# jacobnzw/SSMToybox

Measured on AMD Instinct MI355X. Metric: filter steps/sec (batched MC) for GPQ-Kalman UNGM, higher is better.
Workload: dtype f64; 1 GPU; GPQ-Kalman (GaussianProcessTransform, RBF, UT points) on UNGM, D=1, N=3, 10000 MC trajectories per GPU x T=100 per pass (BASELINE configs[1]); mc_per_gpu=10000, mc_total=10000, parallelism=mc-shard x1, collective=SingleComm, devices=1 x  (gfx950:sramecc+:xnack-, 256 CUs) [0000:8e:00.0], distinct_devices=1, comm_world=1

## Files before the change

include/ssmq.h:

```cpp
#ifndef SSMQ_H
#define SSMQ_H

#ifndef __HIPCC_RTC__
#include <stddef.h>
#include <stdint.h>
#endif

#ifdef __cplusplus
extern "C" {
#endif

#define SSMQ_VERSION 102

#define SSMQ_OK 0
#define SSMQ_E_ARG (-1)
#define SSMQ_E_HIP (-2)
#define SSMQ_E_UNSUPPORTED (-3)
#define SSMQ_E_NOMEM (-4)

#define SSMQ_MAX_FPAR 16
#define SSMQ_MAX_FIDX 16
#define SSMQ_MAX_DIM 16
#define SSMQ_MAX_PTS 4096

// ... 256 lines not shown
                      const int32_t *d_status, const double *mse, double *sums);

int ssmq_traj_scores_rows(int D);
int ssmq_traj_scores_dev(int D, int64_t B, int64_t ld, int T, int k0, const double *d_x, const double *d_fm, const double *d_fP,
                         const int32_t *d_status, const double *mse, double *d_scores);

int ssmq_bootstrap_var_dev(const double *d_data, int64_t ld, int R, const int32_t *d_idx, int64_t n, int S, uint64_t seed,
                           double *var, double *d_means);
int ssmq_bootstrap_var(const double *data, int64_t n, int S, uint64_t seed, double *var);

int ssmq_mc_transform_dev(const ssmq_integrand *f, int D, int E, int64_t n, uint64_t seed, int64_t B, int64_t ld,
                          const double *d_mean, const double *d_cov, const double *d_time, int time_stride, double *d_mean_f,
                          double *d_cov_f, double *d_cov_fx, int32_t *d_status);
int ssmq_mc_unit_points(int D, uint64_t seed, int64_t first, int64_t count, double *z);

int ssmq_kl_divergence_dev(int E, int64_t B, int64_t ld, const double *d_m0, const double *d_P0, int bcast0, const double *d_m1,
                           const double *d_P1, int symmetrized, double *d_kl, int32_t *d_status);

int ssmq_student_filter_forward_dev(ssmq_transform *h_dyn, const ssmq_integrand *f_dyn, ssmq_transform *h_obs,
                                    const ssmq_integrand *f_obs, int64_t B, int64_t ld, int T, const double *d_y,
                                    const double *d_m0, const double *d_S0, const double *GqG, const double *r_smat,
                                    const double *scale, double dof, double *d_fm, double *d_fP, int32_t *d_status);

typedef struct ssmq_filter_job {
    ssmq_transform *h_dyn;
    const ssmq_integrand *f_dyn;
    ssmq_transform *h_obs;
    const ssmq_integrand *f_obs;
    int64_t B, ld;
    int32_t T, reserved;
    const double *d_y, *d_m0, *d_P0;
    const double *GQG, *R;
    double *d_fm, *d_fP;
    int32_t *d_status;
    const double *scale;
    double dof;
} ssmq_filter_job;
int ssmq_filter_forward_multi_dev(int n_jobs, const ssmq_filter_job *jobs);

#define SSMQ_PIPED_OUT_PINNED 1
#define SSMQ_PIPED_X0_PER_TRAJECTORY 2
int ssmq_filter_forward_piped(ssmq_transform *h_dyn, const ssmq_integrand *f_dyn, ssmq_transform *h_obs,
                              const ssmq_integrand *f_obs, int64_t B, int T, const double *y, const double *m0,
                              const double *P0, const double *GQG, const double *R, double *fm, double *fP,
                              int32_t *status, int flags, int n_blocks);
int ssmq_pinned_alloc(size_t bytes, void **p);
int ssmq_pinned_free(void *p);
int ssmq_pinned_is_block(const void *p);

int ssmq_filter_kernel_name(const ssmq_transform *h_dyn, const ssmq_integrand *f_dyn, const ssmq_transform *h_obs,
                            const ssmq_integrand *f_obs, char *buf, int len);
int ssmq_filter_kernel_name_batch(const ssmq_transform *h_dyn, const ssmq_integrand *f_dyn, const ssmq_transform *h_obs,
                                  const ssmq_integrand *f_obs, int64_t B, char *buf, int len);

int ssmq_filter_innovations_dev(ssmq_transform *h_dyn, const ssmq_integrand *f_dyn, ssmq_transform *h_obs,
                                const ssmq_integrand *f_obs, int64_t B, int64_t ld, int T, const double *d_y, const double *d_m0,
                                const double *d_P0, const double *d_fm, const double *d_fP, const double *GQG, const double *R,
                                double *d_ymean, double *d_S, double *d_nis, double *d_ll, double *d_total, int32_t *d_status);
int ssmq_innovations_kernel_name(const ssmq_transform *h_dyn, const ssmq_integrand *f_dyn, const ssmq_transform *h_obs,
                                 const ssmq_integrand *f_obs, int64_t B, char *buf, int len);

#define SSMQ_ITERATED_MAX 64
#define SSMQ_ITERATED_LAUNCH_LOOP 1
int ssmq_filter_iterated_dev(ssmq_transform *h_dyn, const ssmq_integrand *f_dyn, ssmq_transform *h_obs, const ssmq_integrand *f_obs,
                             int64_t B, int64_t ld, int T, int iterations, int flags, const double *d_y, const double *d_m0,
                             const double *d_P0, const double *GQG, const double *R, double *d_fm, double *d_fP,
                             double *d_delta , int32_t *d_status);
int ssmq_iterated_kernel_name(const ssmq_transform *h_dyn, const ssmq_integrand *f_dyn, const ssmq_transform *h_obs,
                              const ssmq_integrand *f_obs, int64_t B, int iterations, int flags, char *buf, int len);

int ssmq_smoother_iterated_dev(ssmq_transform *h_dyn, const ssmq_integrand *f_dyn, ssmq_transform *h_obs, const ssmq_integrand *f_obs,
                               int64_t B, int64_t ld, int T, const double *d_y, const double *d_m0, const double *d_P0,
                               const double *GQG, const double *R, int iterations, int flags,
                               const double *d_lin_m , const double *d_lin_P ,
                               double *d_fm, double *d_fP, double *d_sm, double *d_sP, double *d_sm0 ,
                               double *d_sP0 , double *d_delta , int32_t *d_status);
int ssmq_smoother_iterated_kernel_name(const ssmq_transform *h_dyn, const ssmq_integrand *f_dyn, const ssmq_transform *h_obs,
                                       const ssmq_integrand *f_obs, int iterations, char *buf, int len);

#define SSMQ_SWEEP_GP 0
#define SSMQ_SWEEP_BS 1
int ssmq_filter_sweep_dev(const ssmq_integrand *f_dyn, const ssmq_integrand *f_obs, int kind_dyn, int kind_obs, const double *xi_dyn,
                          int N_dyn, const double *xi_obs, int N_obs, const int32_t *mulind_dyn, int NB_dyn, const int32_t *mulind_obs,
                          int NB_obs, const double *par_dyn, const double *par_obs, int P, double jitter_dyn, double jitter_obs, int D,
                          int Y, int64_t B, int64_t ld, int T, const double *d_y, const double *x0_mean, const double *x0_cov,
                          const double *GQG, const double *R, double *d_loglik_total, double *d_nis_mean, double *d_loglik_steps,
                          int32_t *d_status, int32_t *theta_status);
int ssmq_filter_sweep_kernel_name(const ssmq_integrand *f_dyn, const ssmq_integrand *f_obs, int kind_dyn, int kind_obs, int N_dyn,
                                  int N_obs, int D, int Y, char *buf, int len);

int ssmq_student_scores_dev(ssmq_transform *h_dyn, const ssmq_integrand *f_dyn, ssmq_transform *h_obs, const ssmq_integrand *f_obs,
                            int64_t B, int64_t ld, int T, const double *d_y, const double *x0_mean, const double *x0_smat,
                            const double *GqG, const double *r_smat, const double *scale, double dof, double *d_nis, double *d_loglik,
                            double *d_loglik_total, double *d_nis_mean, int32_t *d_status);
int ssmq_student_scores_kernel_name(const ssmq_transform *h_dyn, const ssmq_integrand *f_dyn, const ssmq_transform *h_obs,
                                    const ssmq_integrand *f_obs, char *buf, int len);

#define SSMQ_RECURSION_GAUSS 0
#define SSMQ_RECURSION_STUDENT 1
int ssmq_filter_sweep_t_dev(const ssmq_integrand *f_dyn, const ssmq_integrand *f_obs, int recursion, const double *xi_dyn, int N_dyn,
                            const double *xi_obs, int N_obs, const double *par_dyn, const double *par_obs, const double *nu_dyn,
                            const double *nu_obs, const double *dof, int P, double jitter_dyn, double jitter_obs, int D, int Y, int64_t B,
                            int64_t ld, int T, const double *d_y, const double *x0_mean, const double *x0_mat, const double *GQG,
                            const double *R, const double *scale, double *d_loglik_total, double *d_nis_mean, double *d_loglik_steps,
                            int32_t *d_status, int32_t *theta_status);
int ssmq_filter_sweep_t_kernel_name(const ssmq_integrand *f_dyn, const ssmq_integrand *f_obs, int recursion, int N_dyn, int N_obs, int D,
// ... 63 lines not shown
```

ssmtoybox_amd/_lib.py:

```python
import ctypes
import os

import numpy as np

c_double_p = ctypes.POINTER(ctypes.c_double)
c_int32_p = ctypes.POINTER(ctypes.c_int32)

ABI_VERSION = 102
SSMQ_MAX_FPAR = 16
SSMQ_MAX_FIDX = 16
FORM_BQ, FORM_SIGMA = 0, 1
FORM_BQ_MO = 3
FORM_TAYLOR_GPQD = 4
FORM_TRUNC_SIGMA = 5
FORM_GPQD = 6
EMV_DIAG, EMV_BROADCAST = 0, 1

F_UNGM_DYN, F_UNGM_MEAS, F_UNGMNA_DYN, F_UNGMNA_MEAS = 1, 2, 3, 4
F_PENDULUM_DYN, F_PENDULUM_MEAS, F_REENTRY1D_DYN, F_RANGE_MEAS = 5, 6, 7, 8
F_REENTRY2D_DYN, F_RADAR2D_MEAS, F_CT_DYN, F_BEARING_MEAS = 9, 10, 11, 12
F_CTRS_DYN, F_CV_DYN, F_REENTRY2D_BIAS_DYN, F_SMOOTH10D_DYN = 13, 14, 15, 16
F_USER_FIRST, F_USER_SLOTS, USER_BODY_MAX, USER_MAX_D, USER_MAX_Y = 1024, 64, 8192, 6, 4
RTC_FILTER, RTC_APPLY, RTC_MC, RTC_LINEAR, RTC_TAYLOR_GPQD, RTC_GPQD, RTC_INNOVATION, RTC_ITERATED = 0, 1, 2, 3, 4, 5, 6, 7
RTC_SMOOTHER_ITERATED = 8
# ... 194 lines not shown
    'ssmq_particle_filter_dev': (ctypes.c_int, [ctypes.POINTER(Integrand), ctypes.POINTER(Integrand), ctypes.c_int, ctypes.c_int, ctypes.c_int,
                                                ctypes.c_int, ctypes.c_int64, ctypes.c_int64, ctypes.c_int] + [ctypes.c_void_p] * 3 +
                                 [c_double_p, c_double_p, c_double_p, ctypes.POINTER(Rv), ctypes.c_double, ctypes.c_uint64, ctypes.c_uint64] +
                                 [ctypes.c_void_p] * 8),
    'ssmq_particle_kernel_name': (ctypes.c_int, [ctypes.POINTER(Integrand), ctypes.POINTER(Integrand), ctypes.c_int, ctypes.c_int, ctypes.c_int,
                                                 ctypes.c_int, ctypes.POINTER(Rv), ctypes.c_char_p, ctypes.c_int]),
    'ssmq_particle_smoother_dev': (ctypes.c_int, [ctypes.POINTER(Integrand), ctypes.c_int, ctypes.c_int, ctypes.c_int, ctypes.c_int64,
                                                  ctypes.c_int64, ctypes.c_int, c_double_p, c_double_p, c_double_p, ctypes.c_int] +
                                   [ctypes.c_void_p] * 13),
    'ssmq_particle_smoother_kernel_name': (ctypes.c_int, [ctypes.POINTER(Integrand), ctypes.c_int, ctypes.c_int, ctypes.c_int, c_double_p,
                                                          c_double_p, c_double_p, ctypes.c_int, ctypes.c_char_p, ctypes.c_int]),
    'ssmq_particle_filter_rv_dev': (ctypes.c_int, [ctypes.POINTER(Integrand), ctypes.POINTER(Integrand), ctypes.c_int, ctypes.c_int, ctypes.c_int,
                                                   ctypes.c_int, ctypes.c_int64, ctypes.c_int64, ctypes.c_int] + [ctypes.c_void_p] * 3 +
                                    [ctypes.POINTER(Rv), ctypes.POINTER(Rv), c_double_p, ctypes.POINTER(Rv), ctypes.c_double, ctypes.c_uint64,
                                     ctypes.c_uint64] + [ctypes.c_void_p] * 8),
    'ssmq_particle_kernel_name_rv': (ctypes.c_int, [ctypes.POINTER(Integrand), ctypes.POINTER(Integrand), ctypes.c_int, ctypes.c_int, ctypes.c_int,
                                                    ctypes.c_int, ctypes.POINTER(Rv), ctypes.POINTER(Rv), ctypes.POINTER(Rv), ctypes.c_char_p,
                                                    ctypes.c_int]),
    'ssmq_particle_smoother_rv_dev': (ctypes.c_int, [ctypes.POINTER(Integrand), ctypes.c_int, ctypes.c_int, ctypes.c_int, ctypes.c_int64,
                                                     ctypes.c_int64, ctypes.c_int, ctypes.POINTER(Rv), c_double_p, ctypes.c_int] +
                                      [ctypes.c_void_p] * 13),
    'ssmq_particle_smoother_kernel_name_rv': (ctypes.c_int, [ctypes.POINTER(Integrand), ctypes.c_int, ctypes.c_int, ctypes.c_int,
                                                             ctypes.POINTER(Rv), c_double_p, ctypes.c_int, ctypes.c_char_p, ctypes.c_int]),
    'ssmq_pcrlb_sums_width': (ctypes.c_int, [ctypes.c_int]),
    'ssmq_pcrlb_sums_dev': (ctypes.c_int, [ctypes.POINTER(Integrand), ctypes.POINTER(Integrand), ctypes.c_int, ctypes.c_int, ctypes.c_int,
                                           ctypes.c_int64, ctypes.c_int64, ctypes.c_int, ctypes.c_void_p, ctypes.POINTER(Rv), c_double_p,
                                           ctypes.POINTER(Rv), c_double_p]),
    'ssmq_pcrlb_kernel_name': (ctypes.c_int, [ctypes.POINTER(Integrand), ctypes.POINTER(Integrand), ctypes.c_int, ctypes.c_int, ctypes.c_int,
                                              ctypes.POINTER(Rv), c_double_p, ctypes.POINTER(Rv), ctypes.c_char_p, ctypes.c_int]),
    'ssmq_pcrlb_finalize': (ctypes.c_int, [ctypes.c_int, ctypes.c_int, ctypes.c_int64, c_double_p, c_double_p, ctypes.POINTER(Rv), c_double_p,
                                           c_double_p, c_double_p, c_double_p, c_int32_p]),
    'ssmq_error_sums_width': (ctypes.c_int, [ctypes.c_int]),
    'ssmq_error_sums_dev': (ctypes.c_int, [ctypes.c_int, ctypes.c_int64, ctypes.c_int64, ctypes.c_int, ctypes.c_void_p,
                                           ctypes.c_void_p, ctypes.c_void_p, ctypes.c_void_p, c_double_p]),
    'ssmq_lcr_sums_dev': (ctypes.c_int, [ctypes.c_int, ctypes.c_int64, ctypes.c_int64, ctypes.c_int, ctypes.c_void_p,
                                         ctypes.c_void_p, ctypes.c_void_p, ctypes.c_void_p, c_double_p, c_double_p]),
    'ssmq_traj_scores_rows': (ctypes.c_int, [ctypes.c_int]),
    'ssmq_traj_scores_dev': (ctypes.c_int, [ctypes.c_int, ctypes.c_int64, ctypes.c_int64, ctypes.c_int, ctypes.c_int, ctypes.c_void_p,
                                            ctypes.c_void_p, ctypes.c_void_p, ctypes.c_void_p, c_double_p, ctypes.c_void_p]),
    'ssmq_bootstrap_var_dev': (ctypes.c_int, [ctypes.c_void_p, ctypes.c_int64, ctypes.c_int, ctypes.c_void_p, ctypes.c_int64,
                                              ctypes.c_int, ctypes.c_uint64, c_double_p, ctypes.c_void_p]),
    'ssmq_bootstrap_var': (ctypes.c_int, [c_double_p, ctypes.c_int64, ctypes.c_int, ctypes.c_uint64, c_double_p]),
    'ssmq_mc_transform_dev': (ctypes.c_int, [ctypes.POINTER(Integrand), ctypes.c_int, ctypes.c_int, ctypes.c_int64, ctypes.c_uint64,
                                             ctypes.c_int64, ctypes.c_int64, ctypes.c_void_p, ctypes.c_void_p, ctypes.c_void_p,
                                             ctypes.c_int, ctypes.c_void_p, ctypes.c_void_p, ctypes.c_void_p, ctypes.c_void_p]),
    'ssmq_mc_unit_points': (ctypes.c_int, [ctypes.c_int, ctypes.c_uint64, ctypes.c_int64, ctypes.c_int64, c_double_p]),
    'ssmq_kl_divergence_dev': (ctypes.c_int, [ctypes.c_int, ctypes.c_int64, ctypes.c_int64, ctypes.c_void_p, ctypes.c_void_p,
                                              ctypes.c_int, ctypes.c_void_p, ctypes.c_void_p, ctypes.c_int, ctypes.c_void_p,
                                              ctypes.c_void_p]),
    'ssmq_filter_kernel_name': (ctypes.c_int, [ctypes.c_void_p, ctypes.POINTER(Integrand), ctypes.c_void_p,
                                               ctypes.POINTER(Integrand), ctypes.c_char_p, ctypes.c_int]),
    'ssmq_filter_kernel_name_batch': (ctypes.c_int, [ctypes.c_void_p, ctypes.POINTER(Integrand), ctypes.c_void_p,
                                                     ctypes.POINTER(Integrand), ctypes.c_int64, ctypes.c_char_p, ctypes.c_int]),
    'ssmq_filter_innovations_dev': (ctypes.c_int, [ctypes.c_void_p, ctypes.POINTER(Integrand), ctypes.c_void_p, ctypes.POINTER(Integrand),
                                                   ctypes.c_int64, ctypes.c_int64, ctypes.c_int] + [ctypes.c_void_p] * 5 +
                                    [c_double_p, c_double_p] + [ctypes.c_void_p] * 6),
    'ssmq_innovations_kernel_name': (ctypes.c_int, [ctypes.c_void_p, ctypes.POINTER(Integrand), ctypes.c_void_p,
                                                    ctypes.POINTER(Integrand), ctypes.c_int64, ctypes.c_char_p, ctypes.c_int]),
    'ssmq_filter_sweep_dev': (ctypes.c_int, [ctypes.POINTER(Integrand), ctypes.POINTER(Integrand), ctypes.c_int, ctypes.c_int,
                                             c_double_p, ctypes.c_int, c_double_p, ctypes.c_int, c_int32_p, ctypes.c_int, c_int32_p,
                                             ctypes.c_int, c_double_p, c_double_p, ctypes.c_int, ctypes.c_double, ctypes.c_double,
                                             ctypes.c_int, ctypes.c_int, ctypes.c_int64, ctypes.c_int64, ctypes.c_int, ctypes.c_void_p] +
                              [c_double_p] * 4 + [ctypes.c_void_p] * 4 + [c_int32_p]),
    'ssmq_filter_sweep_kernel_name': (ctypes.c_int, [ctypes.POINTER(Integrand), ctypes.POINTER(Integrand)] + [ctypes.c_int] * 6 +
                                      [ctypes.c_char_p, ctypes.c_int]),
    'ssmq_student_scores_dev': (ctypes.c_int, [ctypes.c_void_p, ctypes.POINTER(Integrand), ctypes.c_void_p, ctypes.POINTER(Integrand),
                                               ctypes.c_int64, ctypes.c_int64, ctypes.c_int, ctypes.c_void_p] + [c_double_p] * 5 +
                                [ctypes.c_double] + [ctypes.c_void_p] * 5),
    'ssmq_student_scores_kernel_name': (ctypes.c_int, [ctypes.c_void_p, ctypes.POINTER(Integrand), ctypes.c_void_p,
                                                       ctypes.POINTER(Integrand), ctypes.c_char_p, ctypes.c_int]),
    'ssmq_filter_sweep_t_dev': (ctypes.c_int, [ctypes.POINTER(Integrand), ctypes.POINTER(Integrand), ctypes.c_int, c_double_p, ctypes.c_int,
                                               c_double_p, ctypes.c_int] + [c_double_p] * 5 +
                                [ctypes.c_int, ctypes.c_double, ctypes.c_double, ctypes.c_int, ctypes.c_int, ctypes.c_int64, ctypes.c_int64,
                                 ctypes.c_int, ctypes.c_void_p] + [c_double_p] * 5 + [ctypes.c_void_p] * 4 + [c_int32_p]),
    'ssmq_filter_sweep_t_kernel_name': (ctypes.c_int, [ctypes.POINTER(Integrand), ctypes.POINTER(Integrand)] + [ctypes.c_int] * 5 +
                                        [ctypes.c_char_p, ctypes.c_int]),
    'ssmq_filter_noise_sweep_dev': (ctypes.c_int, [ctypes.c_void_p, ctypes.POINTER(Integrand), ctypes.c_void_p, ctypes.POINTER(Integrand),
                                                   ctypes.c_int, ctypes.c_int64, ctypes.c_int64, ctypes.c_int, ctypes.c_void_p, ctypes.c_int] +
                                    [c_double_p, ctypes.c_int64] * 3 + [ctypes.c_void_p] * 4),
    'ssmq_filter_noise_sweep_kernel_name': (ctypes.c_int, [ctypes.c_void_p, ctypes.POINTER(Integrand), ctypes.c_void_p,
                                                           ctypes.POINTER(Integrand), ctypes.c_int, ctypes.c_char_p, ctypes.c_int]),
    'ssmq_filter_iterated_dev': (ctypes.c_int, [ctypes.c_void_p, ctypes.POINTER(Integrand), ctypes.c_void_p, ctypes.POINTER(Integrand),
                                                ctypes.c_int64, ctypes.c_int64, ctypes.c_int, ctypes.c_int, ctypes.c_int] +
                                 [ctypes.c_void_p] * 3 + [c_double_p, c_double_p] + [ctypes.c_void_p] * 4),
    'ssmq_iterated_kernel_name': (ctypes.c_int, [ctypes.c_void_p, ctypes.POINTER(Integrand), ctypes.c_void_p, ctypes.POINTER(Integrand),
                                                 ctypes.c_int64, ctypes.c_int, ctypes.c_int, ctypes.c_char_p, ctypes.c_int]),
    'ssmq_smoother_iterated_dev': (ctypes.c_int, [ctypes.c_void_p, ctypes.POINTER(Integrand), ctypes.c_void_p, ctypes.POINTER(Integrand),
                                                  ctypes.c_int64, ctypes.c_int64, ctypes.c_int] + [ctypes.c_void_p] * 3 +
                                   [c_double_p, c_double_p, ctypes.c_int, ctypes.c_int] + [ctypes.c_void_p] * 10),
    'ssmq_smoother_iterated_kernel_name': (ctypes.c_int, [ctypes.c_void_p, ctypes.POINTER(Integrand), ctypes.c_void_p,
                                                          ctypes.POINTER(Integrand), ctypes.c_int, ctypes.c_char_p, ctypes.c_int]),
    'ssmq_rbf_eval': (ctypes.c_int, [ctypes.c_int, ctypes.c_int, c_double_p, ctypes.c_int, c_double_p, c_double_p,
                                     ctypes.c_int, ctypes.c_int, ctypes.c_int, c_double_p]),
    'ssmq_rbf_factor': (ctypes.c_int, [ctypes.c_int, ctypes.c_int, c_double_p, c_double_p, ctypes.c_int, ctypes.c_int,
                                       ctypes.c_double, c_double_p, c_double_p, c_double_p, c_int32_p]),
    'ssmq_rbf_exp_kxkx': (ctypes.c_int, [ctypes.c_int, ctypes.c_int, c_double_p, c_double_p, c_double_p, ctypes.c_int,
                                         c_double_p]),
    'ssmq_rbf_student_expect': (ctypes.c_int, [ctypes.c_int, ctypes.c_int, c_double_p, c_double_p, c_double_p, ctypes.c_double,
                                               ctypes.c_int64, ctypes.c_uint64, c_double_p, c_double_p, c_double_p]),
    'ssmq_rbf_student_kxy': (ctypes.c_int, [ctypes.c_int, c_double_p, ctypes.c_double, ctypes.c_int64, ctypes.c_uint64,
                                            c_double_p, c_double_p]),
    'ssmq_weights_gp_given': (ctypes.c_int, [ctypes.c_int, ctypes.c_int, c_double_p, c_double_p, ctypes.c_double, c_double_p,
                                             c_double_p, c_double_p, ctypes.c_double] + [c_double_p] * 6 + [c_int32_p]),
    'ssmq_bs_moments': (ctypes.c_int, [ctypes.c_int, ctypes.c_int, c_double_p, c_double_p, c_int32_p, ctypes.c_int,
                                       c_double_p, c_double_p, c_double_p, c_double_p, c_double_p]),
    'ssmq_current_device': (ctypes.c_int, []),
# ... 403 lines not shown
```

ssmtoybox_amd/csrc/ssmq_api_filter.hip:

```cpp
#include <algorithm>
#include <cstring>
#include <vector>
#include "ssmq_host.h"
#include "ssmq_fused.h"

using namespace ssmq;

namespace {
struct DevBuf {
    void *p = nullptr;
    ~DevBuf() { if (p) hipFree(p); }
    int alloc(size_t bytes) { return hip_fail(hipMalloc(&p, bytes ? bytes : 8), "hipMalloc"); }
    double *d() { return (double *)p; }
};
}

extern "C" {
int ssmq_kalman_update_dev(int D, int Y, int64_t B, int64_t ld, const double *d_m_pr, const double *d_P_pr,
                           const double *d_y_mean, const double *d_P_y, const double *d_P_yx, const double *d_y,
                           double *d_m_fi, double *d_P_fi, int32_t *d_status) {
    if (D < 1 || Y < 1 || B < 0 || ld < B || !d_m_pr || !d_P_pr || !d_y_mean || !d_P_y || !d_P_yx || !d_y || !d_m_fi ||
        !d_P_fi || !d_status)
        return SSMQ_E_ARG;
    if (D > SSMQ_MAX_DIM || Y > SSMQ_MAX_DIM) {
// ... 475 lines not shown
        return SSMQ_E_ARG;
    }
    int rc = ensure_device();
    if (rc) return rc;
    if (B == 0) return SSMQ_OK;
    if (T == 0) {
        if (d_status) SSMQ_HIP(hipMemsetAsync(d_status, 0, sizeof(int32_t) * ld, stream()));
        SSMQ_HIP(hipStreamSynchronize(stream()));
        return SSMQ_OK;
    }
    const int D = h_dyn->D;
    DevBuf pm, pP, pC;
    if ((rc = pm.alloc(sizeof(double) * (size_t)T * D * ld)) || (rc = pP.alloc(sizeof(double) * (size_t)T * D * D * ld)) ||
        (rc = pC.alloc(sizeof(double) * (size_t)T * D * D * ld)))
        return rc;
    GraphDropGuard drop_on_exit;
    rc = filter_forward_impl(h_dyn, f_dyn, h_obs, f_obs, B, ld, T, d_y, d_m0, d_P0, GQG, R, d_fm, d_fP, d_status,
                             nullptr, 0.0, pm.d(), pP.d(), pC.d());
    if (rc) return rc;
    rc = launch_rts_backward(D, B, ld, T, d_fm, d_fP, pm.d(), pP.d(), pC.d(), d_sm, d_sP, d_status, stream(), D);
    if (rc) {
        hipStreamSynchronize(stream());
        return rc;
    }
    SSMQ_HIP(hipStreamSynchronize(stream()));
    return SSMQ_OK;
}

extern "C" int ssmq_student_filter_forward_dev(ssmq_transform *h_dyn, const ssmq_integrand *f_dyn,
                                               ssmq_transform *h_obs, const ssmq_integrand *f_obs, int64_t B,
                                               int64_t ld, int T, const double *d_y, const double *d_m0,
                                               const double *d_S0, const double *GqG, const double *r_smat,
                                               const double *scale, double dof, double *d_fm, double *d_fP,
                                               int32_t *d_status) {
    SSMQ_HANDLE_LOCK(h_dyn, h_obs);
    if (is_mo(h_dyn) || is_mo(h_obs)) return refuse_mo("ssmq_student_filter_forward_dev");
    if (is_trunc(h_dyn) || is_trunc(h_obs)) return refuse_trunc("ssmq_student_filter_forward_dev");
    if (is_gpqd(h_dyn) || is_gpqd(h_obs)) return refuse_gpqd("ssmq_student_filter_forward_dev");
    if (!scale || !(dof > 0.0)) {
        set_error("student_filter_forward: scale[T] and dof > 0 are required");
        return SSMQ_E_ARG;
    }
    return filter_forward_impl(h_dyn, f_dyn, h_obs, f_obs, B, ld, T, d_y, d_m0, d_S0, GqG, r_smat, d_fm, d_fP, d_status,
                               scale, dof);
}

extern "C" int ssmq_filter_kernel_name(const ssmq_transform *h_dyn, const ssmq_integrand *f_dyn,
                                       const ssmq_transform *h_obs, const ssmq_integrand *f_obs, char *buf, int len) {
    return ssmq_filter_kernel_name_batch(h_dyn, f_dyn, h_obs, f_obs, 0, buf, len);
}

extern "C" int ssmq_filter_kernel_name_batch(const ssmq_transform *h_dyn, const ssmq_integrand *f_dyn, const ssmq_transform *h_obs,
                                             const ssmq_integrand *f_obs, int64_t B, char *buf, int len) {
    SSMQ_HANDLE_LOCK(h_dyn, h_obs);
    if (!h_dyn || !h_obs || !f_dyn || !f_obs || !buf || len <= 0 || B < 0) return SSMQ_E_ARG;
    const char *name = nullptr;
    FilterPass query;
    int rc = make_filter_pass(h_dyn, f_dyn, h_obs, f_obs, B, 0, 0, nullptr, nullptr, nullptr, nullptr, nullptr, nullptr, nullptr, &query);
    if (rc) return rc;
    query.name = &name; query.dry_run = true;
    const bool mo = is_mo(h_dyn) || is_mo(h_obs);
    if (mo && (is_user_integrand(f_dyn) || is_user_integrand(f_obs))) return refuse_user_integrand("multi-output transform (k_apply_mo)");
    const bool ekf = (h_dyn->form == SSMQ_FORM_TAYLOR1 || is_taylor_gpqd(h_dyn)) && (h_obs->form == SSMQ_FORM_TAYLOR1 || is_taylor_gpqd(h_obs));
    const bool user = is_user_integrand(f_dyn) || is_user_integrand(f_obs);
    if (is_trunc(h_dyn)) return refuse_trunc("filter with a truncated DYNAMICS transform");
    if (is_trunc(h_obs) && h_dyn->form != SSMQ_FORM_SIGMA) return refuse_trunc("filter whose dynamics transform is not a sigma-point rule");
    if (is_trunc(h_obs) && user) return refuse_user_integrand("truncated sigma-point transform (k_apply_trunc)");
    const bool gq = is_gpqd(h_dyn) || is_gpqd(h_obs);
    if (gq && !(is_gpqd(h_dyn) && is_gpqd(h_obs))) return refuse_gpqd("filter with only one GPQ+D transform");
    rc = mo || gq || is_trunc(h_obs) || (user && ekf) || (ssmq::sw("SSMQ_NO_FUSED") && !user) ? 0 : try_launch_fused(query);
    if (rc < 0) return rc;
    snprintf(buf, len, "%s", rc == 1 ? name : "hipGraph of 3 T launches (apply dyn | apply obs | k_kalman_update)");
    return SSMQ_OK;
}

static const char kInnovLoopName[] = "launch loop of 3 T launches (apply dyn | apply obs | k_innovation_score)";
static int innovations_route(const ssmq_transform *h_dyn, const ssmq_integrand *f_dyn, const ssmq_transform *h_obs,
                             const ssmq_integrand *f_obs, PairForms *pf, bool *user_ekf, bool *one_launch) {
    if (is_trunc(h_dyn)) return refuse_trunc("innovation scores with a truncated DYNAMICS transform");
    if (h_dyn->E != h_dyn->D || h_obs->D != h_dyn->D) {
        set_error("filter_innovations: additive-noise Gaussian recursion only (dyn D -> D, obs D -> Y): models that take their noise as an "
                  "argument are not implemented");
        return SSMQ_E_UNSUPPORTED;
    }
    if (int rc = pair_forms(h_dyn, f_dyn, h_obs, f_obs, false, false, pf)) return rc;
    *user_ekf = pf->user && ((jac_form(h_dyn) && jac_form(h_obs)) || pf->gq);
    *one_launch = (pf->user && !*user_ekf) || (!ssmq::sw("SSMQ_NO_FUSED") && !pf->user && !pf->mo && !pf->trunc && !pf->gq);
    return SSMQ_OK;
}

extern "C" int ssmq_filter_innovations_dev(ssmq_transform *h_dyn, const ssmq_integrand *f_dyn, ssmq_transform *h_obs,
                                           const ssmq_integrand *f_obs, int64_t B, int64_t ld, int T, const double *d_y,
                                           const double *d_m0, const double *d_P0, const double *d_fm, const double *d_fP,
                                           const double *GQG, const double *R, double *d_ymean, double *d_S, double *d_nis,
                                           double *d_ll, double *d_total, int32_t *d_status) {
    SSMQ_HANDLE_LOCK(h_dyn, h_obs);
    if (!h_dyn || !h_obs || !f_dyn || !f_obs || B < 0 || ld < B || T < 0 || !d_y || !d_m0 || !d_P0 || !d_fm || !d_fP || !d_nis ||
        !d_ll || !d_total || !d_status) {
        set_error("filter_innovations: bad argument");
        return SSMQ_E_ARG;
    }
    PairForms pf;
    bool user_ekf = false, one_launch = false;
    int rc = innovations_route(h_dyn, f_dyn, h_obs, f_obs, &pf, &user_ekf, &one_launch);
    if (rc) return rc;
    const int D = h_dyn->D, Y = h_obs->E;
    if ((rc = ensure_device())) return rc;
    if (B == 0) return SSMQ_OK;
    hipStream_t s = stream();
    if (T == 0) {
        SSMQ_HIP(hipMemsetAsync(d_status, 0, sizeof(int32_t) * ld, s));
// ... 420 lines not shown
```

ssmtoybox_amd/csrc/ssmq_filter_fused_kernel.h:

```cpp
#pragma once
#ifndef __HIPCC_RTC__
#include <cstdlib>
#endif
#include "ssmq_fused.h"
#include "ssmq_quad.h"
#ifndef __HIPCC_RTC__
#include <type_traits>
#include "ssmq_host.h"
#endif

namespace ssmq {

#ifdef SSMQ_FUSED_NO_STORE
#undef SSMQ_STORE
#define SSMQ_STORE(dst, v) asm volatile("" ::"v"(v))
#endif
#ifdef SSMQ_FUSED_PLAIN_STORE
#undef SSMQ_STORE
#define SSMQ_STORE(dst, v) (dst) = (v)
#endif
#ifndef SSMQ_FUSED_FORCE_OCC
#define SSMQ_FUSED_FORCE_OCC 0
#endif
#ifndef SSMQ_FUSED_OCC_D5_SIGMA
#define SSMQ_FUSED_OCC_D5_SIGMA 1
#endif
template <int D, int Y, int ND, int NO, int FD, int FO, int FORM, int TP, int SELO, int OPT, int STU, bool CHUNKED, bool QUAD = false>
__device__ __forceinline__ void fused_pass(const FusedArgs &a, uint32_t blk, int k_begin, int k_end, bool first, bool last) {
    static_assert(!QUAD || (D == 1 && !CHUNKED), "fused_pass: the quad form is for whole passes of scalar states");
    const uint32_t b = QUAD ? blk * kQuadTraj + (threadIdx.x >> 2) : blk * a.lpw + threadIdx.x;
    if ((int64_t)b >= a.B) return;
    const int64_t ld = a.ld;
    double m[D], Pl[D * (D + 1) / 2];
    if (!CHUNKED || first) {
#pragma unroll
        for (int d = 0; d < D; ++d) m[d] = a.m0[d * ld + b];
#pragma unroll
        for (int i = 0; i < D; ++i)
#pragma unroll
            for (int j = 0; j <= i; ++j) Pl[SSMQ_PK(i, j)] = a.P0[(i * D + j) * ld + b];
    } else {
        const double *h = a.hand + (size_t)blk * (D + D * (D + 1) / 2 + 1) * 64 + threadIdx.x;
#pragma unroll
        for (int d = 0; d < D; ++d) m[d] = __hip_atomic_load(h + d * 64, __ATOMIC_RELAXED, __HIP_MEMORY_SCOPE_SYSTEM);
#pragma unroll
        for (int i = 0; i < D * (D + 1) / 2; ++i) Pl[i] = __hip_atomic_load(h + (D + i) * 64, __ATOMIC_RELAXED, __HIP_MEMORY_SCOPE_SYSTEM);
    }
    CoreParams cpd{(cdouble_p)a.c_dyn, (cdouble_p)a.gqg, a.emv_dyn, a.nu_dyn, 1.0, 1.0};
    CoreParams cpo{(cdouble_p)a.c_obs, (cdouble_p)a.rr, a.emv_obs, a.nu_obs, 1.0, 1.0};
    const cdouble_p ssc = (cdouble_p)a.sscale;
    const bool stu_scale = STU < 0 ? ssc != nullptr : STU == 1;
    const bool stu_update = STU < 0 ? a.student_dof > 0.0 : STU == 1;
    constexpr bool kScalar = (D == 1 && Y == 1);
    const double nan = __builtin_nan("");
    int32_t agg = 0;
    if (CHUNKED && !first)
        agg = (int32_t)__hip_atomic_load(a.hand + (size_t)blk * (D + D * (D + 1) / 2 + 1) * 64 + (D + D * (D + 1) / 2) * 64 + threadIdx.x, __ATOMIC_RELAXED,
                                         __HIP_MEMORY_SCOPE_SYSTEM);
#ifndef SSMQ_FUSED_YAHEAD
#define SSMQ_FUSED_YAHEAD 1
#endif
    constexpr int YA = SSMQ_FUSED_YAHEAD;
    double ynext[YA][Y];
#pragma unroll
    for (int q = 0; q < YA; ++q)
#pragma unroll
        for (int i = 0; i < Y; ++i) ynext[q][i] = a.y[((int64_t)(k_begin + q < a.T ? k_begin + q : a.T - 1) * Y + i) * ld + b];
    FPar fd = a.fd, fo = a.fo;
    constexpr bool kTTd = HasTimeTable<FD>::value, kTTo = HasTimeTable<FO>::value;
    const cdouble_p ttd = (cdouble_p)a.fd.ttab, tto = (cdouble_p)a.fo.ttab;
    double tdn = 0.0, ton = 0.0, scn = 1.0;
    if constexpr (kTTd) { tdn = ttd[k_begin]; fd.use_tval = 1; }
    if constexpr (kTTo) { ton = tto[k_begin]; fo.use_tval = 1; }
    if (stu_scale) scn = ssc[k_begin];
    QuadScalarPoints<ND> qpts;
    if constexpr (QUAD) qpts.init(cpd.c + const_layout(D, D, ND, FORM).xi, (int)(threadIdx.x & 3));
#pragma unroll
    for (int d = 0; d < D; ++d) pin_v(m[d]);
#pragma unroll
    for (int i = 0; i < D * (D + 1) / 2; ++i) pin_v(Pl[i]);
#pragma unroll
    for (int q = 0; q < YA; ++q)
#pragma unroll
        for (int i = 0; i < Y; ++i) pin_v(ynext[q][i]);
#pragma unroll 1
    for (int k = k_begin; k < k_end; ++k) {
        const double t = (double)k;
        double ycur[Y];
#pragma unroll
        for (int i = 0; i < Y; ++i) ycur[i] = ynext[0][i];
#pragma unroll
        for (int q = 0; q + 1 < YA; ++q)
#pragma unroll
            for (int i = 0; i < Y; ++i) ynext[q][i] = ynext[q + 1][i];
        if constexpr (kTTd) fd.tval = tdn;
        if constexpr (kTTo) fo.tval = ton;
        const double sc = scn;
        {
            const int kn = (k + 1 < a.T) ? k + 1 : k;
            const int ky = YA == 1 ? kn : ((k + YA < a.T) ? k + YA : a.T - 1);
#pragma unroll
            for (int i = 0; i < Y; ++i) ynext[YA - 1][i] = a.y[((int64_t)ky * Y + i) * ld + b];
            if constexpr (kTTd) tdn = ttd[kn];
            if constexpr (kTTo) ton = tto[kn];
            if (stu_scale) scn = ssc[kn];
        }
        if (stu_scale) {
            cpd.cov_scale = sc;
            cpo.cov_scale = sc;
            cpo.ccov_scale = sc;
        }
        RegSinkNoCross<D, D> pr;
        bool ok;
        if constexpr (QUAD) ok = moment_transform_core<D, D, ND, FD, FORM, TP, 0, false, OPT>(m, Pl, t, fd, cpd, pr, qpts);
        else ok = moment_transform_core<D, D, ND, FD, FORM, TP, 0, false, OPT, RegSinkNoCross<D, D>>(m, Pl, t, fd, cpd, pr);
        double L2[D * (D + 1) / 2];
#pragma unroll
        for (int i = 0; i < D * (D + 1) / 2; ++i) L2[i] = pr.cv[i];
        RegSink<D, Y> ob;
        ok = moment_transform_core<D, Y, NO, FO, FORM, TP, SELO, true, OPT, RegSink<D, Y>>(pr.mf, L2, t, fo, cpo, ob) && ok;
        double S[Y * (Y + 1) / 2];
#pragma unroll
        for (int i = 0; i < Y * (Y + 1) / 2; ++i) S[i] = ob.cv[i];
        double G[D][Y];
        constexpr bool kPoisonRow = !kScalar;
        if (kPoisonRow && Y > 1) {
            ok = chol_packed<Y>(S) && ok;
        } else if (kPoisonRow) {
            ok = (S[0] > 0.0) && ok;
        }
        if (kPoisonRow) {
            if (agg == 0 && !ok) agg = k + 1;
#pragma unroll
            for (int d = 0; d < D; ++d) ob.cx[0][d] = (agg == 0) ? ob.cx[0][d] : nan;
        }
        if (Y == 1) {
            if constexpr (kScalar) {
                int hi = __double2hiint(S[0]);
                hi = (S[0] > 0.0) ? hi : 0x7ff80000;
                S[0] = __hiloint2double(hi, __double2loint(S[0]));
            }
#pragma unroll
            for (int d = 0; d < D; ++d) G[d][0] = div_nr(ob.cx[0][d], S[0]);
        } else {
#pragma unroll
            for (int d = 0; d < D; ++d) {
                double v[Y];
#pragma unroll
                for (int i = 0; i < Y; ++i) {
                    double s = ob.cx[i][d];
#pragma unroll
                    for (int q = 0; q < i; ++q) s -= S[SSMQ_PK(i, q)] * v[q];
                    v[i] = div_nr(s, S[SSMQ_PK(i, i)]);
                }
#pragma unroll
                for (int i = Y - 1; i >= 0; --i) {
                    double s = v[i];
#pragma unroll
                    for (int q = i + 1; q < Y; ++q) s -= S[SSMQ_PK(q, i)] * v[q];
                    v[i] = div_nr(s, S[SSMQ_PK(i, i)]);
                }
#pragma unroll
                for (int i = 0; i < Y; ++i) G[d][i] = v[i];
            }
        }
        const bool good = true;
        double sc2 = 1.0;
        if (stu_update) {
// ... 70 lines not shown
```

ssmtoybox_amd/csrc/ssmq_filter_ungm_quad.hip:

```cpp
#include "ssmq_filter_fused_kernel.h"

namespace ssmq {
namespace {

template <int N>
__global__ __launch_bounds__(kSmallBlock, 2) void k_filter_ungm_quad(const FusedArgs a) {
    fused_pass<1, 1, N, N, SSMQ_F_UNGM_DYN, SSMQ_F_UNGM_MEAS, SSMQ_FORM_BQ, 0, 0, 0, 0, false, true>(a, blockIdx.x, 0, a.T, true, true);
}

typedef void (*ungm_quad_kernel)(const FusedArgs);
struct UngmQuadEntry {
    int N;
    ungm_quad_kernel k;
    const char *name;
};
#define SSMQ_UQ(N) {N, &k_filter_ungm_quad<N>, "k_filter_ungm_quad<N=" #N ",SSMQ_FORM_BQ,TP=0>"}
const UngmQuadEntry kUngmQuad[] = {SSMQ_UQ(2), SSMQ_UQ(3), SSMQ_UQ(5)};

}

int try_launch_ungm_quad(const FilterPass &p, int64_t waves) {
    const ssmq_transform *hd = p.hd, *ho = p.ho;
    if (p.fd->id != SSMQ_F_UNGM_DYN || p.fo->id != SSMQ_F_UNGM_MEAS || hd->D != 1 || hd->E != 1 || ho->D != 1 || ho->E != 1) return 0;
    if (hd->form != SSMQ_FORM_BQ || hd->tp_nu > 0.0 || ho->N != hd->N || p.sel_obs != 0) return 0;
    if (!p.ttab_dyn && !p.dry_run) return 0;
    for (const UngmQuadEntry &e : kUngmQuad) {
        if (e.N != hd->N) continue;
        if (p.name) *p.name = e.name;
        if (p.dry_run) return 1;
        FusedArgs a = fused_args(p);
        a.lpw = kQuadTraj;
        hipLaunchKernelGGL(e.k, dim3((unsigned)waves), dim3(kSmallBlock), 0, p.s, a);
        const int rc = hip_fail(hipGetLastError(), e.name);
        return rc ? rc : 1;
    }
    return 0;
}

}
```

ssmtoybox_amd/ssinf.py:

```python
import ctypes

import numpy as np

from . import _lib
from .mtran import (MomentTransform, LinearizationTransform, TaylorGPQDTransform, UnscentedTransform, SphericalRadialTransform, GaussHermiteTransform,
                    FullySymmetricStudentTransform, TruncatedUnscentedTransform, TruncatedSphericalRadialTransform,
                    TruncatedGaussHermiteTransform, resolve_integrand)
from .bq.bqmtran import (GaussianProcessTransform, BayesSardTransform, StudentTProcessTransform,
                         MultiOutputGaussianProcessTransform, GaussianProcessDerTransform)
from .ssmod import TransitionModel, MeasurementModel, is_user_model, has_device_jacobian, user_unsupported, check_user_points


_NOT_PD = 'Matrix is not positive definite (trajectory {}, step {})'


def _raise_failed(status, prefix='', message=_NOT_PD):
    if status.any():
        b = int(np.flatnonzero(status)[0])
        raise np.linalg.LinAlgError(prefix + message.format(b, int(status[b]) - 1))


def _iteration_count(iterations):
    if isinstance(iterations, bool) or int(iterations) != iterations or not 1 <= int(iterations) <= _lib.ITERATED_MAX:
        raise ValueError('iterations must be an integer in 1 .. {} (got {!r})'.format(_lib.ITERATED_MAX, iterations))
# ... 74 lines not shown
        self.fi_mean = self.fi_cov = None
        self.sm_mean = self.sm_cov = None
        self.status = None
        self._data = None

    def reset(self):
        self.fi_mean = self.fi_cov = None
        self.sm_mean = self.sm_cov = None
        self.status = None
        self._data = None

    def _check_user_points(self):
        if is_user_model(self.mod_dyn) or is_user_model(self.mod_obs):
            for tf in (self.tf_dyn, self.tf_obs):
                if tf._num_points():
                    check_user_points(self.mod_dyn.dim_state, tf._num_points())

    @property
    def _additive(self):
        return self.mod_dyn.noise_additive and self.mod_obs.noise_additive

    _recursion = 'gauss'

    def _pair(self):
        f_dyn, e_dyn = resolve_integrand(self.mod_dyn.dyn_eval)
        f_obs, e_obs = resolve_integrand(self.mod_obs.meas_eval)
        return self.tf_dyn._handle_for(e_dyn), f_dyn, self.tf_obs._handle_for(e_obs), f_obs

    def _noise(self):
        gqg = np.ascontiguousarray(self.G.dot(self.q_cov).dot(self.G.T), dtype=np.float64) if self.mod_dyn.noise_additive else None
        rr = np.ascontiguousarray(self.r_cov, dtype=np.float64) if self.mod_obs.noise_additive else None
        return gqg, rr

    def _noise_aug(self):
        def moments(mean, cov):
            mean = np.ascontiguousarray(np.atleast_1d(mean), dtype=np.float64)
            return mean, np.ascontiguousarray(np.atleast_2d(cov), dtype=np.float64), int(mean.shape[0])
        gqg, rr = self._noise()
        return ((None, gqg, 0) if gqg is not None else moments(self.q_mean, self.q_cov)) + \
               ((None, rr, 0) if rr is not None else moments(self.r_mean, self.r_cov))

    def _kernel_name(self, fn, *extra, unsupported=False):
        buf = ctypes.create_string_buffer(512)
        _lib.check(getattr(_lib.load(), fn)(*self._pair(), *extra, buf, 512), fn, unsupported)
        return buf.value.decode()

    def _initial_planes(self, stage, B, ld, x0_mean=None, x0_cov=None, broadcast_on_device=False):
        return initial_planes(stage, self.mod_dyn.dim_state, self.x0_mean, self._initial_cov(), B, ld, x0_mean, x0_cov,
                              broadcast_on_device)

    def _initial_cov(self):
        return self.x0_cov

    def kernel_name(self, batch=0):
        if not self._additive:
            return ('k_filter_fused_aug (one kernel for the time loop) where instantiated, else a launch loop of 5 T '
                    'launches (k_augment | apply dyn | k_augment | apply obs | k_kalman_update)')
        self._check_user_points()
        return self._kernel_name('ssmq_filter_kernel_name_batch', int(batch))

    def forward_pass(self, data):
        fm, fP = self.forward_pass_batch(np.asarray(data)[..., None])
        return fm[..., 0], fP[..., 0]

    def _launch(self, lib, B, ld, T, d_y, d_m0, d_P0, d_fm, d_fP, d_st):
        if not self._additive:
            return self._launch_aug(lib, B, ld, T, d_y, d_m0, d_P0, d_fm, d_fP, d_st)
        gqg, rr = self._noise()
        vp, dp = _lib.vp, _lib.dp
        _lib.check(lib.ssmq_filter_forward_dev(*self._pair(), B, ld, T, vp(d_y), vp(d_m0), vp(d_P0), dp(gqg), dp(rr), vp(d_fm), vp(d_fP),
                                               vp(d_st)), 'ssmq_filter_forward_dev')

    def _launch_smooth(self, lib, B, ld, T, d_y, d_m0, d_P0, d_fm, d_fP, d_sm, d_sP, d_st):
        if not self._additive:
            return self._launch_aug(lib, B, ld, T, d_y, d_m0, d_P0, d_fm, d_fP, d_st, d_sm, d_sP)
        gqg, rr = self._noise()
        vp, dp = _lib.vp, _lib.dp
        _lib.check(lib.ssmq_filter_smooth_dev(*self._pair(), B, ld, T, vp(d_y), vp(d_m0), vp(d_P0), dp(gqg), dp(rr), vp(d_fm), vp(d_fP),
                                              vp(d_sm), vp(d_sP), vp(d_st)), 'ssmq_filter_smooth_dev')

    def _launch_aug(self, lib, B, ld, T, d_y, d_m0, d_P0, d_fm, d_fP, d_st, d_sm=None, d_sP=None):
        qm, qc, dq, rm, rc, dr = self._noise_aug()
        vp, dp = _lib.vp, _lib.dp
        args = (*self._pair(), self.mod_dyn.dim_state, B, ld, T, vp(d_y), vp(d_m0), vp(d_P0), dp(qm), dp(qc), dq, dp(rm), dp(rc), dr,
                vp(d_fm), vp(d_fP))
        if d_sm is not None:
            _lib.check(lib.ssmq_filter_smooth_aug_dev(*args, vp(d_sm), vp(d_sP), vp(d_st)), 'ssmq_filter_smooth_aug_dev')
        else:
            _lib.check(lib.ssmq_filter_forward_aug_dev(*args, vp(d_st)), 'ssmq_filter_forward_aug_dev')

    def backward_pass(self):
        sm, sP = self.backward_pass_batch()
        return sm[..., 0], sP[..., 0]

    def backward_pass_batch(self):
        assert self._data is not None, 'run forward_pass first'
        if is_user_model(self.mod_dyn) or is_user_model(self.mod_obs):
            raise user_unsupported('the RTS smoother (backward_pass)')
        self.forward_pass_batch(self._data, smooth=True)
        return self.sm_mean, self.sm_cov

    def forward_pass_dev(self, d_y, B, ld, T):
        self._check_user_points()
        lib = _lib.load()
        D = self.mod_dyn.dim_state
        with _lib.Staging() as stage:
            d_m0, d_P0 = self._initial_planes(stage, B, ld, broadcast_on_device=True)
            d_fm, d_fP, d_st = stage.device(8 * T * D * ld), stage.device(8 * T * D * D * ld), stage.device(4 * ld)
            self._launch(lib, B, ld, T, d_y, d_m0, d_P0, d_fm, d_fP, d_st)
            _lib.sync()
            return stage.release(d_fm, d_fP, d_st)
# ... 1630 lines not shown
```

Before: 32.27 billion filter steps/s.

## Specialize UNGM quad filter kernel with 32-bit offsets and prefetched loads

Replaces the generic fused_pass call in the scalar UNGM quad kernel with a dedicated loop that unrolls two steps per iteration. It keeps byte offsets in 32-bit registers, prefetches the next observation and t-table value ahead of the current step, and counts NaN-free steps for the status word instead of checking them separately. The aim is to cut address arithmetic and hide memory latency in the serial time loop. The dispatcher now rejects shapes whose offsets would overflow 32 bits, and a shape-aware kernel-name query is added so callers can see that fallback.

```diff
diff --git a/include/ssmq.h b/include/ssmq.h
--- a/include/ssmq.h
+++ b/include/ssmq.h
@@ -332,6 +332,8 @@
                             const ssmq_integrand *f_obs, char *buf, int len);
 int ssmq_filter_kernel_name_batch(const ssmq_transform *h_dyn, const ssmq_integrand *f_dyn, const ssmq_transform *h_obs,
                                   const ssmq_integrand *f_obs, int64_t B, char *buf, int len);
+int ssmq_filter_kernel_name_shape(const ssmq_transform *h_dyn, const ssmq_integrand *f_dyn, const ssmq_transform *h_obs,
+                                  const ssmq_integrand *f_obs, int64_t B, int64_t ld, int T, char *buf, int len);
 
 int ssmq_filter_innovations_dev(ssmq_transform *h_dyn, const ssmq_integrand *f_dyn, ssmq_transform *h_obs,
                                 const ssmq_integrand *f_obs, int64_t B, int64_t ld, int T, const double *d_y, const double *d_m0,
diff --git a/ssmtoybox_amd/_lib.py b/ssmtoybox_amd/_lib.py
--- a/ssmtoybox_amd/_lib.py
+++ b/ssmtoybox_amd/_lib.py
@@ -270,6 +270,9 @@
                                                ctypes.POINTER(Integrand), ctypes.c_char_p, ctypes.c_int]),
     'ssmq_filter_kernel_name_batch': (ctypes.c_int, [ctypes.c_void_p, ctypes.POINTER(Integrand), ctypes.c_void_p,
                                                      ctypes.POINTER(Integrand), ctypes.c_int64, ctypes.c_char_p, ctypes.c_int]),
+    'ssmq_filter_kernel_name_shape': (ctypes.c_int, [ctypes.c_void_p, ctypes.POINTER(Integrand), ctypes.c_void_p,
+                                                     ctypes.POINTER(Integrand), ctypes.c_int64, ctypes.c_int64, ctypes.c_int,
+                                                     ctypes.c_char_p, ctypes.c_int]),
     'ssmq_filter_innovations_dev': (ctypes.c_int, [ctypes.c_void_p, ctypes.POINTER(Integrand), ctypes.c_void_p, ctypes.POINTER(Integrand),
                                                    ctypes.c_int64, ctypes.c_int64, ctypes.c_int] + [ctypes.c_void_p] * 5 +
                                     [c_double_p, c_double_p] + [ctypes.c_void_p] * 6),
diff --git a/ssmtoybox_amd/csrc/ssmq_api_filter.hip b/ssmtoybox_amd/csrc/ssmq_api_filter.hip
--- a/ssmtoybox_amd/csrc/ssmq_api_filter.hip
+++ b/ssmtoybox_amd/csrc/ssmq_api_filter.hip
@@ -551,11 +551,16 @@
 
 extern "C" int ssmq_filter_kernel_name_batch(const ssmq_transform *h_dyn, const ssmq_integrand *f_dyn, const ssmq_transform *h_obs,
                                              const ssmq_integrand *f_obs, int64_t B, char *buf, int len) {
-    SSMQ_HANDLE_LOCK(h_dyn, h_obs);
-    if (!h_dyn || !h_obs || !f_dyn || !f_obs || !buf || len <= 0 || B < 0) return SSMQ_E_ARG;
+    return ssmq_filter_kernel_name_shape(h_dyn, f_dyn, h_obs, f_obs, B, 0, 0, buf, len);
+}
+
+extern "C" int ssmq_filter_kernel_name_shape(const ssmq_transform *h_dyn, const ssmq_integrand *f_dyn, const ssmq_transform *h_obs,
+                                             const ssmq_integrand *f_obs, int64_t B, int64_t ld, int T, char *buf, int len) {
+    SSMQ_HANDLE_LOCK(h_dyn, h_obs);
+    if (!h_dyn || !h_obs || !f_dyn || !f_obs || !buf || len <= 0 || B < 0 || ld < 0 || T < 0 || (ld > 0 && ld < B)) return SSMQ_E_ARG;
     const char *name = nullptr;
     FilterPass query;
-    int rc = make_filter_pass(h_dyn, f_dyn, h_obs, f_obs, B, 0, 0, nullptr, nullptr, nullptr, nullptr, nullptr, nullptr, nullptr, &query);
+    int rc = make_filter_pass(h_dyn, f_dyn, h_obs, f_obs, B, ld, T, nullptr, nullptr, nullptr, nullptr, nullptr, nullptr, nullptr, &query);
     if (rc) return rc;
     query.name = &name; query.dry_run = true;
     const bool mo = is_mo(h_dyn) || is_mo(h_obs);
diff --git a/ssmtoybox_amd/csrc/ssmq_filter_fused_kernel.h b/ssmtoybox_amd/csrc/ssmq_filter_fused_kernel.h
--- a/ssmtoybox_amd/csrc/ssmq_filter_fused_kernel.h
+++ b/ssmtoybox_amd/csrc/ssmq_filter_fused_kernel.h
@@ -25,10 +25,9 @@
 #ifndef SSMQ_FUSED_OCC_D5_SIGMA
 #define SSMQ_FUSED_OCC_D5_SIGMA 1
 #endif
-template <int D, int Y, int ND, int NO, int FD, int FO, int FORM, int TP, int SELO, int OPT, int STU, bool CHUNKED, bool QUAD = false>
+template <int D, int Y, int ND, int NO, int FD, int FO, int FORM, int TP, int SELO, int OPT, int STU, bool CHUNKED>
 __device__ __forceinline__ void fused_pass(const FusedArgs &a, uint32_t blk, int k_begin, int k_end, bool first, bool last) {
-    static_assert(!QUAD || (D == 1 && !CHUNKED), "fused_pass: the quad form is for whole passes of scalar states");
-    const uint32_t b = QUAD ? blk * kQuadTraj + (threadIdx.x >> 2) : blk * a.lpw + threadIdx.x;
+    const uint32_t b = blk * a.lpw + threadIdx.x;
     if ((int64_t)b >= a.B) return;
     const int64_t ld = a.ld;
     double m[D], Pl[D * (D + 1) / 2];
@@ -73,8 +72,6 @@
     if constexpr (kTTd) { tdn = ttd[k_begin]; fd.use_tval = 1; }
     if constexpr (kTTo) { ton = tto[k_begin]; fo.use_tval = 1; }
     if (stu_scale) scn = ssc[k_begin];
-    QuadScalarPoints<ND> qpts;
-    if constexpr (QUAD) qpts.init(cpd.c + const_layout(D, D, ND, FORM).xi, (int)(threadIdx.x & 3));
 #pragma unroll
     for (int d = 0; d < D; ++d) pin_v(m[d]);
 #pragma unroll
@@ -111,9 +108,7 @@
             cpo.ccov_scale = sc;
         }
         RegSinkNoCross<D, D> pr;
-        bool ok;
-        if constexpr (QUAD) ok = moment_transform_core<D, D, ND, FD, FORM, TP, 0, false, OPT>(m, Pl, t, fd, cpd, pr, qpts);
-        else ok = moment_transform_core<D, D, ND, FD, FORM, TP, 0, false, OPT, RegSinkNoCross<D, D>>(m, Pl, t, fd, cpd, pr);
+        bool ok = moment_transform_core<D, D, ND, FD, FORM, TP, 0, false, OPT, RegSinkNoCross<D, D>>(m, Pl, t, fd, cpd, pr);
         double L2[D * (D + 1) / 2];
 #pragma unroll
         for (int i = 0; i < D * (D + 1) / 2; ++i) L2[i] = pr.cv[i];
diff --git a/ssmtoybox_amd/csrc/ssmq_filter_ungm_quad.hip b/ssmtoybox_amd/csrc/ssmq_filter_ungm_quad.hip
--- a/ssmtoybox_amd/csrc/ssmq_filter_ungm_quad.hip
+++ b/ssmtoybox_amd/csrc/ssmq_filter_ungm_quad.hip
@@ -3,9 +3,101 @@
 namespace ssmq {
 namespace {
 
+typedef const __attribute__((address_space(4))) char *cbyte_p;
+
+template <int N>
+struct UngmQuadPass {
+    CoreParams cpd, cpo;
+    FPar fd, fo;
+    QuadScalarPoints<N> qpts;
+    const char *ynx;
+    char *fm, *fP;
+    cbyte_p tt;
+    uint32_t pitch;
+    uint32_t vo;
+    uint32_t to;
+    double m[1], Pl[1];
+    double tdn;
+    int32_t agg;
+
+    template <bool AHEAD>
+    __device__ __forceinline__ void step(int k, const double ycur, double &ynext) {
+        const double t = (double)k;
+        fd.tval = tdn;
+        if constexpr (AHEAD) {
+            ynext = *(const double *)(ynx + vo);
+        }
+        RegSinkNoCross<1, 1> pr;
+        bool ok = moment_transform_core<1, 1, N, SSMQ_F_UNGM_DYN, SSMQ_FORM_BQ, 0, 0, false, 0>(m, Pl, t, fd, cpd, pr, qpts);
+        if constexpr (AHEAD) {
+            __builtin_amdgcn_sched_barrier(0);
+            tdn = *(cdouble_p)(tt + to);
+            to += 8;
+        }
+        double L2[1] = {pr.cv[0]};
+        RegSink<1, 1> ob;
+        ok = moment_transform_core<1, 1, N, SSMQ_F_UNGM_MEAS, SSMQ_FORM_BQ, 0, 0, true, 0, RegSink<1, 1>>(pr.mf, L2, t, fo, cpo, ob) && ok;
+        double S = ob.cv[0];
+        int hi = __double2hiint(S);
+        hi = (S > 0.0) ? hi : 0x7ff80000;
+        S = __hiloint2double(hi, __double2loint(S));
+        const double G = div_nr(ob.cx[0][0], S);
+        double s = 0.0;
+        s += G * (ycur - ob.mf[0]);
+        m[0] = pr.mf[0] + s;
+        double w = 0.0;
+        w += G * ob.cv[0];
+        double s2 = 0.0;
+        s2 += w * G;
+        double p = pr.cv[0] - s2;
+        if constexpr (AHEAD) asm volatile("" : "+v"(ynext), "+v"(m[0]), "+v"(p));
+        SSMQ_STORE(*(double *)(fm + vo), m[0]);
+        SSMQ_STORE(*(double *)(fP + vo), p);
+        agg += (p == p) ? 1 : 0;
+        Pl[0] = p;
+        vo += pitch;
+    }
+};
+
 template <int N>
 __global__ __launch_bounds__(kSmallBlock, 2) void k_filter_ungm_quad(const FusedArgs a) {
-    fused_pass<1, 1, N, N, SSMQ_F_UNGM_DYN, SSMQ_F_UNGM_MEAS, SSMQ_FORM_BQ, 0, 0, 0, 0, false, true>(a, blockIdx.x, 0, a.T, true, true);
+    const uint32_t b = blockIdx.x * kQuadTraj + (threadIdx.x >> 2);
+    const int T = a.T;
+    if (b >= (uint32_t)a.B || T < 1) return;
+    UngmQuadPass<N> u;
+    u.cpd = CoreParams{(cdouble_p)a.c_dyn, (cdouble_p)a.gqg, a.emv_dyn, a.nu_dyn, 1.0, 1.0};
+    u.cpo = CoreParams{(cdouble_p)a.c_obs, (cdouble_p)a.rr, a.emv_obs, a.nu_obs, 1.0, 1.0};
+    u.fd = a.fd;
+    u.fo = a.fo;
+    u.fd.use_tval = 1;
+    u.pitch = 8u * (uint32_t)a.ld;
+    u.vo = 8u * b;
+    u.to = 8;
+    u.ynx = (const char *)a.y + u.pitch;
+    u.fm = (char *)a.fm;
+    u.fP = (char *)a.fP;
+    u.tt = (cbyte_p)a.fd.ttab;
+    u.m[0] = *(const double *)((const char *)a.m0 + u.vo);
+    u.Pl[0] = *(const double *)((const char *)a.P0 + u.vo);
+    u.agg = 0;
+    double ya = *(const double *)((const char *)a.y + u.vo), yb;
+    u.tdn = *(cdouble_p)u.tt;
+    u.qpts.init(u.cpd.c + const_layout(1, 1, N, SSMQ_FORM_BQ).xi, (int)(threadIdx.x & 3));
+    pin_v(u.m[0]);
+    pin_v(u.Pl[0]);
+    pin_v(ya);
+    int k = 0;
+#pragma unroll 1
+    for (const uint32_t to_end = 8u * (uint32_t)((T - 1) | 1); u.to != to_end; k += 2) {
+        u.template step<true>(k, ya, yb);
+        u.template step<true>(k + 1, yb, ya);
+    }
+    if (!(T & 1)) {
+        u.template step<true>(k++, ya, yb);
+        ya = yb;
+    }
+    u.template step<false>(k, ya, yb);
+    *(int32_t *)((char *)a.status + 4u * b) = (u.agg == T) ? 0 : u.agg + 1;
 }
 
 typedef void (*ungm_quad_kernel)(const FusedArgs);
@@ -24,6 +116,8 @@
     if (p.fd->id != SSMQ_F_UNGM_DYN || p.fo->id != SSMQ_F_UNGM_MEAS || hd->D != 1 || hd->E != 1 || ho->D != 1 || ho->E != 1) return 0;
     if (hd->form != SSMQ_FORM_BQ || hd->tp_nu > 0.0 || ho->N != hd->N || p.sel_obs != 0) return 0;
     if (!p.ttab_dyn && !p.dry_run) return 0;
+    if (p.ld >= ((int64_t)1 << 28) || 8 * p.ld * p.T >= ((int64_t)1 << 31)) return 0;
+    if (p.T < 1 && !p.dry_run) return 0;
     for (const UngmQuadEntry &e : kUngmQuad) {
         if (e.N != hd->N) continue;
         if (p.name) *p.name = e.name;
diff --git a/ssmtoybox_amd/ssinf.py b/ssmtoybox_amd/ssinf.py
--- a/ssmtoybox_amd/ssinf.py
+++ b/ssmtoybox_amd/ssinf.py
@@ -150,11 +150,13 @@
     def _initial_cov(self):
         return self.x0_cov
 
-    def kernel_name(self, batch=0):
+    def kernel_name(self, batch=0, ld=0, T=0):
         if not self._additive:
             return ('k_filter_fused_aug (one kernel for the time loop) where instantiated, else a launch loop of 5 T '
                     'launches (k_augment | apply dyn | k_augment | apply obs | k_kalman_update)')
         self._check_user_points()
+        if ld or T:
+            return self._kernel_name('ssmq_filter_kernel_name_shape', int(batch), int(ld), int(T))
         return self._kernel_name('ssmq_filter_kernel_name_batch', int(batch))
 
     def forward_pass(self, data):
```

Measured after the change: 36.72 billion filter steps/s (median of 6 runs). +13.8%, better.
